# psipred/DMPfold2

Measured on AMD Instinct MI355X. Metric: structures/s at L=300, N_seq=2000, 10 iters+100 min, higher is better.
Workload: dtype f32 with full-width operands on the bf16 matrix cores (option precision = 2): convolution operands split exactly into 3 bf16 pieces (24 significand bits), the 6 piece products above 2^-24 accumulated in f32 by v_mfma_f32_32x32x16_bf16; vertical GRU the same way (3 bf16 pieces per operand, 6 products

## Files before the change

### dmpfold2_amd/csrc/api.hip

```cpp
#include "common.h"
#include <atomic>
#include "conv_bf16.h"
#include "conv_f16.h"
#include <cstdarg>
#include <cstdio>
#include <cstring>
#include <cmath>

namespace dmp {

static thread_local char g_err[512] = "";

void set_error(const char* fmt, ...) {
  va_list ap;
  va_start(ap, fmt);
  vsnprintf(g_err, sizeof(g_err), fmt, ap);
  va_end(ap);
}

int hip_fail(hipError_t e, const char* what, const char* file, int line) {
  set_error("HIP error %d (%s) at %s:%d: %s", (int)e, hipGetErrorString(e), file, line, what);
  return DMP_ERR_HIP;
}

// ... 208 lines not shown
        sc = std::ldexp(1.0f, std::max(-40, std::min(40, 15 - e)));
      }
      W.blk[k - 1].x_scale = sc;
      const std::string p = "resnet." + std::to_string(k);
      bound += 2.0f * reach(H[p + ".layer1.norm.weight"], H[p + ".layer1.norm.bias"]);
    }
  }
  for (int k = 1; k <= NBLOCK; ++k) {
    const std::string p = "resnet." + std::to_string(k);
    BlockW& B = W.blk[k - 1];
    const auto& w = H[p + ".layer1.lin.weight"];
    std::vector<float> pk((size_t)512 * 128 * 25);
    for (int split = 0; split < CONV_SPLIT; ++split)
      for (int chunk = 0; chunk < CW / CONV_CC; ++chunk)
        for (int tap = 0; tap < 25; ++tap)
          for (int cc = 0; cc < CONV_CC; ++cc)
            for (int m = 0; m < 128; ++m) {
              const int och = split * 128 + m, ich = chunk * CONV_CC + cc;
              pk[((((size_t)split * (CW / CONV_CC) + chunk) * 25 + tap) * CONV_CC + cc) * 128 + m] =
                  w[((size_t)och * 128 + ich) * 25 + tap];
            }
    if ((rc = upload(pool, bytes, &B.wpack, pk))) return rc;
    {
      const std::vector<uint16_t> q = pack_conv_weights_bf16(w.data());
      if ((rc = dev_alloc(pool, bytes, &B.wq, (int64_t)q.size()))) return rc;
      DMP_HIP(hipMemcpy(B.wq, q.data(), sizeof(uint16_t) * q.size(), hipMemcpyHostToDevice));
      const float scale = conv_weight_scale_f16(w.data(), w.size());
      const std::vector<uint16_t> h = pack_conv_weights_f16(w.data(), scale);
      if ((rc = dev_alloc(pool, bytes, &B.wh, (int64_t)h.size()))) return rc;
      DMP_HIP(hipMemcpy(B.wh, h.data(), sizeof(uint16_t) * h.size(), hipMemcpyHostToDevice));
      B.wh_inv_scale = 1.0f / scale;
    }
    if ((rc = upload(pool, bytes, &B.bias, H[p + ".layer1.lin.bias"]))) return rc;
    if ((rc = upload(pool, bytes, &B.gamma, H[p + ".layer1.norm.weight"]))) return rc;
    const auto& beta = H[p + ".layer1.norm.bias"];
    if ((rc = upload(pool, bytes, &B.beta, beta))) return rc;
    const auto& w1 = H[p + ".scSE.cSE.fc.0.weight"];
    const auto& w2 = H[p + ".scSE.cSE.fc.2.weight"];
    std::vector<float> hid(8), gate(128);
    for (int r = 0; r < 8; ++r) {
      float a = 0.f;
      for (int q = 0; q < 128; ++q) a += w1[r * 128 + q] * beta[q];
      hid[r] = a > 0.f ? a : 0.f;
    }
    for (int q = 0; q < 128; ++q) {
      float a = 0.f;
      for (int r = 0; r < 8; ++r) a += w2[q * 8 + r] * hid[r];
      gate[q] = 1.0f / (1.0f + std::exp(-a));
    }
    if ((rc = upload(pool, bytes, &B.cse, gate))) return rc;
    {
      std::vector<float> fc(w1);
      fc.insert(fc.end(), w2.begin(), w2.end());
      if ((rc = upload(pool, bytes, &B.cse_fc, fc))) return rc;
    }
    if ((rc = upload(pool, bytes, &B.sse_w, H[p + ".scSE.sSE.conv.weight"]))) return rc;
    B.sse_b = H[p + ".scSE.sSE.conv.bias"][0];
  }
  if ((rc = upload(pool, bytes, &W.head_w, H["resnet.17.weight"]))) return rc;
  W.head_b[0] = H["resnet.17.bias"][0];
  W.head_b[1] = H["resnet.17.bias"][1];
  return DMP_OK;
}

static int check_ready(dmp_ctx* c, int L, int N) {
  if (!c) { set_error("null context"); return DMP_ERR_ARG; }
  if (L > c->max_L || N > c->max_N) {
    set_error("alignment %d x %d exceeds the context capacity %d x %d", N, L, c->max_N, c->max_L);
    return DMP_ERR_CAPACITY;
  }
  return DMP_OK;
}
static int need_weights(dmp_ctx* c) {
  if (!c->W.ready) { set_error("weights not finalized"); return DMP_ERR_WEIGHTS; }
  return DMP_OK;
}

static int trunk_open(dmp_ctx* c, const float* z0, const float* dmap, int L, hipStream_t s) {
  int rc;
  c->trunk_cur = c->xa;
  c->trunk_oth = c->xb;
  c->xsplit_current = false;
  c->ab_current = false;
  if ((rc = stem_update_padded(c, z0, dmap, L, c->trunk_cur, s, true))) return rc;
  c->xsplit_current = c->conv_mode != 1;
  return DMP_OK;
}

static int trunk_block(dmp_ctx* c, int k, int L, hipStream_t s) {
  int rc;
  {
    static const int depth = getenv("DMP_LANE_DEPTH") ? std::max(1, atoi(getenv("DMP_LANE_DEPTH"))) : 2;
    if (c->lane && c->lane->count >= depth)
      DMP_HIP(hipStreamWaitEvent(s, (hipEvent_t)c->lane->ev[(c->lane->count - depth) % dmp_lane::RING], 0));
  }
  if (c->prof_on && c->prof_n + 2 <= (int)c->prof_ev.size()) {
    DMP_HIP(hipEventRecord((hipEvent_t)c->prof_ev[c->prof_n], s));
  }
  if ((rc = conv5x5_maxout_padded(c, k, c->trunk_cur, L, c->u, c->stats, s, false))) return rc;
  if (c->lane) {
    dmp_lane* ln = c->lane;
    void* e = ln->ev[ln->next];
    ln->next = (ln->next + 1) % dmp_lane::RING;
    DMP_HIP(hipEventRecord((hipEvent_t)e, s));
    ln->last = e;
    ln->count++;
  }
  if (c->prof_on && c->prof_n + 2 <= (int)c->prof_ev.size()) {
    DMP_HIP(hipEventRecord((hipEvent_t)c->prof_ev[c->prof_n + 1], s));
    c->prof_n += 2;
  }
  if ((rc = conv5x5_reduce_stats(c, L, c->stats, s, k))) return rc;
  if ((rc = norm_scse_residual_padded(c, k, c->u, c->stats, c->trunk_cur, L, c->trunk_oth, s, k == NBLOCK))) return rc;
  std::swap(c->trunk_cur, c->trunk_oth);
  return DMP_OK;
}

static int trunk_close(dmp_ctx* c, int L, float* d_conf, float* d_M, hipStream_t s) {
  c->xsplit_current = false;
  return head_gram_padded(c, c->trunk_cur, L, d_conf, d_M, s);
}

static int trunk_pass(dmp_ctx* c, const float* z0, const float* dmap, int L, float* d_conf,
                      float* d_M, hipStream_t s) {
  struct Reset { dmp_ctx* c; ~Reset() { c->xsplit_current = false; } } reset{c};
  int rc;
  if ((rc = trunk_open(c, z0, dmap, L, s))) return rc;
  for (int k = 1; k <= NBLOCK; ++k)
    if ((rc = trunk_block(c, k, L, s))) return rc;
  return trunk_close(c, L, d_conf, d_M, s);
}

static int coords_from_mds(dmp_ctx* c, const float* mat1d, const float* mds, int L, float* d_ca,
                           hipStream_t s) {
  int rc;
  if ((rc = build_embed(mat1d, mds, L, c->emb, s))) return rc;
  if ((rc = gru_bidir(c, 1, c->emb, L, c->seq_a, s))) return rc;
  return coord_fc(c, c->seq_a, L, d_ca, s);
}

__global__ void fault_latch_kernel(int* __restrict__ words, float* __restrict__ coords,
                                   float* __restrict__ conf, int L, ConfLayout lay, int* __restrict__ report) {
  const int f = words[0];
  if (!f) return;
  const int64_t i = (int64_t)blockIdx.x * blockDim.x + threadIdx.x;
  const float nan = __builtin_nanf("");
  if (i < 15 * L) coords[i] = nan;
  if (i < lay.score_off || (i >= lay.score_out && i < lay.align_off) || (i >= lay.ss_off && i < lay.align_off) ||
      (i >= lay.align_out && i < lay.total))
    conf[i] = nan;
  if (i == 0) {
    atomicOr(&words[1], f);
    if (report) *report = f;
  }
}

static int search_reserve(dmp_ctx* c) {
  if (c->opt.search <= 0) return DMP_OK;
  const int mm = c->opt.search_mm > 0 ? c->opt.search_mm : c->max_L;
  int64_t need = 0;
  for (int L = 8; L <= c->max_L; ++L)
    need = std::max<int64_t>(need, (int64_t)search_chunk_entries(L, mm, 0) * search_slot(L, mm).total);
  need += SEARCH_HEAD_BYTES;
  if (c->search_ws && c->search_ws_bytes >= need) return DMP_OK;
  int prev = 0;
  DMP_HIP(hipGetDevice(&prev));
  DMP_HIP(hipSetDevice(c->device));
  void* p = nullptr;
  hipError_t e = hipMalloc(&p, (size_t)need);
  if (e == hipSuccess) e = hipMemset(p, 0, (size_t)SEARCH_HEAD_BYTES);
  if (e == hipSuccess && c->search_ws) e = hipFree(c->search_ws);
  (void)hipSetDevice(prev);
  if (e != hipSuccess) {
    if (p) (void)hipFree(p);
    return hip_fail(e, "search scratch", __FILE__, __LINE__);
  }
  c->bytes += need - c->search_ws_bytes;
  c->search_ws = (unsigned char*)p;
  c->search_ws_bytes = need;
  return DMP_OK;
}

static int passes_reserve(dmp_ctx* c) {
  if (c->pass_ws) return DMP_OK;
  const int64_t need = score_passes_bytes(c->max_L);
  int prev = 0;
  DMP_HIP(hipGetDevice(&prev));
  DMP_HIP(hipSetDevice(c->device));
  void* p = nullptr;
  hipError_t e = hipMalloc(&p, (size_t)need);
  if (e == hipSuccess) e = hipMemset(p, 0, (size_t)score_passes_head_bytes());
  (void)hipSetDevice(prev);
  if (e != hipSuccess) {
    if (p) (void)hipFree(p);
    return hip_fail(e, "pass-score scratch", __FILE__, __LINE__);
  }
  c->bytes += need;
  c->pass_ws = (unsigned char*)p;
  c->pass_ws_bytes = need;
  return DMP_OK;
}

static int ss_reserve(dmp_ctx* c) {
  if (c->ss_ws) return DMP_OK;
  const int64_t need = assign_ss_bytes(c->max_L);
  int prev = 0;
  DMP_HIP(hipGetDevice(&prev));
  DMP_HIP(hipSetDevice(c->device));
// ... 905 lines not shown
    c->vg_index = i;
    c->fe_vgru = i == 0 ? ((n > 1 || (lead->vgru_persist && lead->vgru_persist_ok)) ? 1 : cdiv(maxN + 1, FE_VGRU_STEPS)) : 0;
    c->fe_total = 1 + c->fe_inv + c->fe_vgru + 1;
  }
  return DMP_OK;
}

int dmp_predict_group_riders(dmp_ctx* lead, int n, const uint8_t* const* d_msas, const int* Ns, const int* Ls,
                             float* const* d_outs) {
  DMP_ARG(lead && d_msas && Ns && Ls && d_outs && n >= 1, "bad argument");
  DMP_ARG(lead->vg_leader == lead && lead->fe_next == 0 && lead->vg_riders.empty(),
          "add riders right after dmp_predict_group_vgru, once, before the leader issues a unit");
  DMP_ARG((int)lead->vg_members.size() + n <= 8, "a chain serves at most 8 alignments (%d members + %d riders)",
          (int)lead->vg_members.size(), n);
  int cols = 0, maxN = 0;
  for (dmp_ctx* m : lead->vg_members) { cols += round_up(m->last_L, 32); maxN = std::max(maxN, m->last_N); }
  for (int i = 0; i < n; ++i) {
    DMP_ARG(d_msas[i] && d_outs[i] && Ns[i] >= 1 && Ls[i] >= 8, "bad argument for rider %d", i);
    if (Ls[i] > lead->max_L || Ns[i] > lead->max_N) {
      set_error("rider %d: alignment %d x %d exceeds the context capacity %d x %d", i, Ns[i], Ls[i], lead->max_N, lead->max_L);
      return DMP_ERR_CAPACITY;
    }
    cols += round_up(Ls[i], 32);
    maxN = std::max(maxN, Ns[i]);
  }
  if (cols > lead->vg_cap_cols) {
    set_error("the chain's %d alignment columns exceed the leader's capacity %d", cols, lead->vg_cap_cols);
    return DMP_ERR_CAPACITY;
  }
  for (int i = 0; i < n; ++i) lead->vg_riders.push_back({d_msas[i], Ns[i], Ls[i], d_outs[i]});
  lead->fe_vgru = 1;
  lead->fe_total = 1 + lead->fe_inv + lead->fe_vgru + 1;
  return DMP_OK;
}

int dmp_predict_set_vgru_result(dmp_ctx* ctx, const float* d_vout, void* event) {
  DMP_ARG(ctx && d_vout, "null argument");
  DMP_ARG(ctx->fe_total > 0 && ctx->fe_next == 0 && ctx->vg_leader == nullptr,
          "hand the vertical-GRU result over right after dmp_predict_begin_units, before any unit is issued");
  ctx->ext_vout = d_vout;
  ctx->ext_vout_ev = event;
  ctx->fe_vgru = 0;
  ctx->fe_total = 1 + ctx->fe_inv + 1;
  return DMP_OK;
}

int dmp_predict_next_unit(const dmp_ctx* ctx) {
  if (!ctx) return DMP_UNIT_NONE;
  if (ctx->fe_next == ctx->fe_total - 1 && ctx->vg_leader && ctx->vg_leader != ctx && !vg_done(ctx->vg_leader))
    return DMP_UNIT_WAIT;
  if (ctx->fe_next < ctx->fe_total) return DMP_UNIT_LIGHT;
  if (recycle_gate(const_cast<dmp_ctx*>(ctx), false) == 0) return DMP_UNIT_WAIT;
  if (ctx->passes_done > ctx->run_nloops) return DMP_UNIT_NONE;
  return (ctx->unit_next >= 1 && ctx->unit_next <= NBLOCK) ? DMP_UNIT_CONV : DMP_UNIT_LIGHT;
}

int dmp_predict_issue_unit(dmp_ctx* ctx, void* stream) {
  DMP_ARG(ctx != nullptr, "null context");
  dmp_ctx* c = ctx;
  hipStream_t s = STREAM;
  if (c->fe_next < c->fe_total) return issue_front_end_unit(c, s);
  DMP_ARG(c->passes_done <= c->run_nloops, "all passes of this prediction were already issued");
  {
    const int go = recycle_gate(c, true);
    if (go < 0) return go;
    if (c->passes_done > c->run_nloops) return DMP_OK;
  }
  const int L = c->last_L, pass = c->passes_done, u = c->unit_next;
  int rc = DMP_OK;
  if (u == 0) {
    if (pass > 0) rc = pair_distances(c->ca, L, 1, c->dmap, s);
    if (!rc) rc = trunk_open(c, c->z0, c->dmap, L, s);
  } else if (u <= NBLOCK) {
    rc = trunk_block(c, u, L, s);
  } else {
    rc = trunk_close(c, L, c->conf, c->gram, s);
    if (!rc) rc = eigh_top8(c, c->gram, L, c->mds, s);
    if (!rc) rc = coords_from_mds(c, c->mat1d, c->mds, L, c->ca, s);
    if (!rc && pass == 0 && c->run_refine > 0) rc = refine_coords(c, c->ca, L, c->run_refine, s);
    if (!rc) rc = select_best(c, c->conf, c->ca, L, pass, c->max_passes, s);
    if (!rc && c->run.emit) rc = keep_best_dm(c, L, pass, s);
    if (!rc && c->run.tol_mA > 0) rc = recycle_delta(c, c->ca, L, pass, c->max_passes, s);
  }
  if (rc) { c->xsplit_current = false; return rc; }
  if (u == NBLOCK + 1) { c->unit_next = 0; c->passes_done = pass + 1; }
  else c->unit_next = u + 1;
  return record_unit(c, s);
}

int dmp_ctx_pending(dmp_ctx* ctx) {
  DMP_ARG(ctx != nullptr, "null context");
  if (ctx->unit_seq == 0) return 0;
  hipError_t e = hipEventQuery((hipEvent_t)ctx->unit_ev[(ctx->unit_seq - 1) & 1]);
  if (e == hipSuccess) return 0;
  if (e != hipErrorNotReady) return hip_fail(e, "hipEventQuery", __FILE__, __LINE__);
  if (ctx->unit_seq < 2) return 1;
  e = hipEventQuery((hipEvent_t)ctx->unit_ev[ctx->unit_seq & 1]);
  if (e == hipSuccess) return 1;
  if (e != hipErrorNotReady) return hip_fail(e, "hipEventQuery", __FILE__, __LINE__);
  return 2;
}


static int predict_end_refine(dmp_ctx* ctx, void* stream) {
  DMP_ARG(ctx != nullptr, "null context");
  dmp_ctx* c = ctx;
  DMP_ARG(c->fe_next >= c->fe_total && c->passes_done == c->run_nloops + 1,
          "dmp_predict_end before all passes were issued");
  if (c->end_refined) return DMP_OK;
  hipStream_t s = STREAM;
  const int L = c->last_L;
  int rc;
  DMP_HIP(hipMemcpyAsync(c->best_ca_snapshot, c->best_ca, sizeof(float) * 3 * L,
                         hipMemcpyDeviceToDevice, s));
  if (c->run_refine > 0 && (rc = refine_coords(c, c->best_ca, L, c->run_refine, s))) return rc;
  c->end_refined = true;
  return record_unit(c, s);
}

int dmp_predict_end(dmp_ctx* ctx, float* d_coords, float* d_conf, void* stream) {
  DMP_ARG(ctx && d_coords && d_conf, "null argument");
  dmp_ctx* c = ctx;
  int rc = predict_end_refine(ctx, stream);
  if (rc) return rc;
  hipStream_t s = STREAM;
  const int L = c->last_L;
  rc = ca_to_backbone(c->best_ca, c->best_conf, L, d_coords, d_conf, s);
  if (rc) return rc;
  const int pass_R = c->run.passes ? std::min(c->run_depth + 1, c->max_passes) : 0;
  const ConfLayout lay = conf_layout(L, c->run.emit, c->run.score, c->run.align, c->run.smap, pass_R, c->run.ss);
  if (c->run.emit && (rc = emit_distmap(c, c->best_ca, L, c->passes_done, d_conf + lay.map_off, d_conf + lay.info_off, s))) return rc;
  if (c->run.score && (rc = score_native(c, d_coords, L, d_conf + lay.score_off, s))) return rc;
  if (c->run.smap && (rc = score_map(c, L, d_conf + lay.score_off, d_conf + lay.smap_off, s))) return rc;
  if (pass_R && (rc = score_passes(c, L, pass_R, std::min(c->passes_done, c->max_passes), d_conf + lay.pass_off, s))) return rc;
  if (c->run.ss && (rc = assign_ss(c, d_coords, L, c->run.score ? d_conf + lay.score_off : nullptr, d_conf + lay.ss_off, s))) return rc;
  if (c->run.align && (rc = align_structure(c, d_coords, L, d_conf + lay.align_off, s))) return rc;
  if (c->run.search > 0 && (rc = search_structures(c, d_coords, L, d_conf, lay, s))) return rc;
  hipLaunchKernelGGL(fault_latch_kernel, dim3((unsigned)cdiv64(std::max<int64_t>(15 * L, lay.total), 256)), dim3(256), 0, s,
                     c->seq_abort, d_coords, d_conf, L, lay, c->end_fault_out);
  DMP_LAUNCH_CHECK();
  return DMP_OK;
}

static std::shared_ptr<dmp_lane> lane_create() {
  std::shared_ptr<dmp_lane> l(new dmp_lane(), [](dmp_lane* p) {
    for (void* e : p->ev) (void)hipEventDestroy((hipEvent_t)e);
    delete p;
  });
  for (int i = 0; i < dmp_lane::RING; ++i) {
    hipEvent_t e;
    if (hipEventCreateWithFlags(&e, hipEventDisableTiming) != hipSuccess) return nullptr;
    l->ev.push_back((void*)e);
  }
  return l;
}

int dmp_ctx_share_lane(dmp_ctx* ctx, dmp_ctx* other) {
  DMP_ARG(ctx != nullptr, "null context");
  if (!other) { ctx->lane_hold.reset(); ctx->lane = nullptr; return DMP_OK; }
  DMP_ARG(other != ctx && other->device == ctx->device, "a lane is shared by different contexts of one GPU");
  if (!other->lane_hold) {
    other->lane_hold = lane_create();
    if (!other->lane_hold) { set_error("hipEventCreate failed for the lane"); return DMP_ERR_HIP; }
    other->lane = other->lane_hold.get();
  }
  ctx->lane_hold = other->lane_hold;
  ctx->lane = ctx->lane_hold.get();
  return DMP_OK;
}

int64_t dmp_debug_fetch(dmp_ctx* ctx, const char* name, float* d_dst, int64_t capacity, void* stream) {
  DMP_ARG(ctx && name && d_dst, "null argument");
  const int64_t L = ctx->last_L, N = ctx->last_N;
  const int64_t P = std::min(ctx->passes_done, ctx->max_passes);
  const float* src = nullptr;
  int64_t n = 0;
  const std::string k(name);
  if (k == "w") { src = ctx->w; n = N; }
  else if (k == "contacts") { src = ctx->contacts; n = L * L; }
  else if (k == "mat1d") { src = ctx->mat1d; n = WIDTH * L; }
  else if (k == "conf_means") { src = ctx->conf_means; n = P; }
  else if (k == "ca_pass") { src = ctx->ca_pass; n = P * L * 3; }
  else if (k == "pass_delta") { src = ctx->pass_delta; n = ctx->run.tol_mA > 0 ? P : 0; }
  else if (k == "best_dm") { src = ctx->best_dm; n = ctx->run.emit ? L * L : 0; }
  else if (k == "best_pass") { src = ctx->best_pass; n = 1; }
  else if (k == "best_ca") { src = ctx->best_ca_snapshot; n = L * 3; }
  else if (k == "best_ca_refined") { src = ctx->best_ca; n = L * 3; }
  else if (k == "inv_cov") { src = ctx->cov; n = (int64_t)NS * L * NS * L; }
  else if (k == "mds") { src = ctx->mds; n = L * 8; }
  else if (k == "gram") { src = ctx->gram; n = L * L; }
  else if (k == "vgru_h0" || k == "vgru_h1") {
    const int layer = k == "vgru_h1";
    src = ctx->hT[layer][ctx->vg_maxN & 1];
    n = (int64_t)WIDTH * ctx->vg_ntiles * 32;
  }
  else { set_error("unknown debug tensor %s", name); return DMP_ERR_ARG; }
  if (n > capacity) { set_error("capacity %lld too small for %s (%lld)", (long long)capacity, name, (long long)n); return DMP_ERR_ARG; }
  if (n > 0) DMP_HIP(hipMemcpyAsync(d_dst, src, sizeof(float) * n, hipMemcpyDeviceToDevice, STREAM));
  return n;
}

int dmp_profile_enable(dmp_ctx* ctx, int on, int max_launches) {
  DMP_ARG(ctx != nullptr, "null context");
  ctx->prof_on = on != 0;
  ctx->prof_n = 0;
  while ((int)ctx->prof_ev.size() < 2 * max_launches) {
    hipEvent_t e;
    DMP_HIP(hipEventCreate(&e));
    ctx->prof_ev.push_back((void*)e);
  }
  return DMP_OK;
}


int dmp_profile_conv_intervals(dmp_ctx* ctx, dmp_ctx* ref, float* h_start_ms, float* h_end_ms, int capacity,
                               int* h_launches) {
  DMP_ARG(ctx && ref && h_start_ms && h_end_ms && h_launches, "null argument");
  DMP_ARG(ref->prof_n >= 2, "the reference context has no recorded launch");
  const int n = ctx->prof_n / 2 < capacity ? ctx->prof_n / 2 : capacity;
  hipEvent_t e0 = (hipEvent_t)ref->prof_ev[0];
  for (int i = 0; i < n; ++i) {
    DMP_HIP(hipEventElapsedTime(&h_start_ms[i], e0, (hipEvent_t)ctx->prof_ev[2 * i]));
    DMP_HIP(hipEventElapsedTime(&h_end_ms[i], e0, (hipEvent_t)ctx->prof_ev[2 * i + 1]));
  }
  *h_launches = n;
  return DMP_OK;
}


}
```

### dmpfold2_amd/csrc/common.h

```cpp
#pragma once
#include <hip/hip_runtime.h>
#include <stdint.h>
#include <string>
#include <vector>
#include <map>
#include <algorithm>
#include <memory>
#include "../../include/dmpfold_hip.h"

namespace dmp {

constexpr int WIDTH = 512;
constexpr int HID2 = 256;
constexpr float VGRU_STATE_SCALE = 1024.f;
constexpr int VGRU_CHUNK = 128;
constexpr int VGRU_CHUNK_SMALL = 16;
constexpr int CW = 128;
constexpr int NBLOCK = 16;
constexpr int STEM_OUT = 384;
constexpr int STEM_IN = 955;
constexpr int NS = 21;
constexpr int NUM_DCA = NS * NS + 1;
constexpr int GJ_NB = 128;
constexpr int CONV_TILE = 16;
// ... 147 lines not shown
struct dmp_ctx {
  int device = 0;
  dmp_lane* lane = nullptr;
  std::shared_ptr<dmp_lane> lane_hold;
  int run_nloops = 0, run_refine = 0;
  int run_depth = 0;
  int max_L = 0, max_N = 0;
  int64_t bytes = 0;
  dmp::Weights W;
  std::vector<void*> allocs;

  uint8_t* msa = nullptr;
  uint32_t* msa_words = nullptr;
  int* nbr_count = nullptr;
  float* w = nullptr;
  double* wsum = nullptr;
  float* colmean = nullptr;
  float* xc = nullptr;
  float* cov = nullptr;
  float* gj_p = nullptr;
  float *gj_c = nullptr, *gj_rt = nullptr;
  void* gj_ev[2] = {nullptr, nullptr};
  int gj_pairs = 1;
  int gj_lookahead = 1;
  int fe_inv_blocks = 6;
  float* contacts = nullptr;
  float* x3 = nullptr;
  double* apc_sums = nullptr;
  float* hT[2][2] = {{nullptr, nullptr}, {nullptr, nullptr}};
  uint16_t* hH[2][2] = {{nullptr, nullptr}, {nullptr, nullptr}};
  uint8_t* vgru_run = nullptr;
  uint8_t* vgru_sync = nullptr;
  uint8_t* vgru_wq = nullptr;
  int vgru_persist = 1;
  bool vgru_persist_ok = false;
  int vgru_debug_drop_wg = 0;
  int vgru_f32 = 2;
  int vg_ntiles = 0, vg_maxN = 0;
  int vg_tile0[8] = {0};
  int vg_cap_cols = 0;
  dmp_ctx* vg_leader = nullptr;
  std::vector<dmp_ctx*> vg_members;
  struct VgRider { const uint8_t* msa; int N, L; float* out; };
  std::vector<VgRider> vg_riders;
  int vg_index = 0;
  bool vg_done_issued = false;
  int vg_waiters = 0;
  void* vg_done_ev = nullptr;
  const float* ext_vout = nullptr;
  void* ext_vout_ev = nullptr;
  std::map<int64_t, void*> vgru_graphs;
  std::map<int, void*> tri_graphs;
  int cluster_local = 1;
  int tridiag_single = 0;
  int tridiag_cluster = 1;
  unsigned long long* tri_gx = nullptr;
  int refine_single = 0;
  int gj_diag_groups = 4;
  int gj_diag_blocked = 0;
  float* vout = nullptr;
  float* seq_g = nullptr;
  float* seq_a = nullptr;
  float* seq_b = nullptr;
  float* emb = nullptr;
  float* mat1d = nullptr;
  unsigned long long* seq_hx = nullptr;
  int* seq_abort = nullptr;
  unsigned long long* refine_gx = nullptr;
  int refine_xcd = 0;
  int seq_xcd0 = 0;
  float* z0 = nullptr;
  float* planes = nullptr;
  int planes_L = 0;
  bool planes_live = false;
  float* dmap = nullptr;
  float* u = nullptr;
  float* xa = nullptr;
  float* xb = nullptr;
  float* xdense = nullptr;
  uint16_t* xsplit = nullptr;
  int conv_mode = 2;
  int act_scaling = 1;
  bool xsplit_current = false;
  bool ab_current = false;
  double* part = nullptr;
  int part_count = 0;
  int conv_tile_bands = 0;
  double* stats = nullptr;
  float* ab = nullptr;
  float* bwd_ws = nullptr;
  int64_t bwd_ws_floats = 0;
  int bwd_w_block = 0;
  float* head0 = nullptr;
  float* head1 = nullptr;
  bool head_current = false;
  float* conf = nullptr;
  float* gram = nullptr;
  double* eig_a = nullptr;
  double* eig_ws = nullptr;
  float* mds = nullptr;
  float* ca = nullptr;
  float* best_ca = nullptr;
  float* best_conf = nullptr;
  float* best_mean = nullptr;
  float* conf_means = nullptr;
  float* ca_pass = nullptr;
  float* best_ca_snapshot = nullptr;
  int passes_done = 0;
  TailOpts opt;
  TailOpts run;
  int gate_pass = 0;
  float* delta_keep = nullptr;
  float* pass_delta = nullptr;
  double* delta_partial = nullptr;
  unsigned* delta_counter = nullptr;
  int* delta_host = nullptr;
  float* best_pass = nullptr;
  float* best_dm = nullptr;
  double* rms_partial = nullptr;
  unsigned* rms_counter = nullptr;
  float* score_pm = nullptr;
  float* score_qn = nullptr;
  int* score_idx = nullptr;
  double* score_hdr = nullptr;
  double* score_rec = nullptr;
  unsigned long long* score_tot = nullptr;
  unsigned* score_ticket = nullptr;
  unsigned* map_cnt = nullptr;
  double* map_partial = nullptr;
  double* map_sums = nullptr;
  unsigned* map_ticket = nullptr;
  float* align_pm = nullptr;
  float* align_qs = nullptr;
  double* align_hdr = nullptr;
  double* align_rec = nullptr;
  int* align_surv = nullptr;
  double* align_btm = nullptr;
  int* align_bali = nullptr;
  unsigned char* align_dir = nullptr;
  unsigned* align_ticket = nullptr;
  unsigned char* search_ws = nullptr;
  int64_t search_ws_bytes = 0;
  int search_last_L = 0, search_last_mm = 0, search_last_C = 0;
  unsigned char* pass_ws = nullptr;
  int64_t pass_ws_bytes = 0;
  unsigned char* ss_ws = nullptr;
  int64_t ss_ws_bytes = 0;
  int* end_fault_out = nullptr;
  bool end_refined = false;
  int unit_next = 0;
  float *trunk_cur = nullptr, *trunk_oth = nullptr;
  void* unit_ev[2] = {nullptr, nullptr};
  void* side_stream = nullptr;
  void* side_ev[2] = {nullptr, nullptr};
  bool fe_side = false;
  long unit_seq = 0;
  int fe_next = 0, fe_total = 0;
  int fe_inv = 0, fe_vgru = 0;
  const uint8_t* run_msa = nullptr;
  const float* run_template = nullptr;
  int last_L = 0, last_N = 0;
  int max_passes = 0;
  bool prof_on = false;
  int prof_n = 0;
  std::vector<void*> prof_ev;
};
// ... 211 lines not shown
```

### dmpfold2_amd/csrc/trunk.hip

```cpp
#include "common.h"
#include <type_traits>
#define CONV_BF16_KERNELS
#include "conv_bf16.h"
#define CONV_F16_KERNELS
#include "conv_f16.h"

#pragma clang fp contract(off)

namespace dmp {

typedef float f32x16 __attribute__((ext_vector_type(16)));

__device__ __forceinline__ float sigmoid_f(float x) { return 1.0f / (1.0f + expf(-x)); }

template <int MODE>
__device__ __forceinline__ void store_pieces(const float (&o)[8], uint16_t* __restrict__ xs, int64_t slot,
                                             int64_t piece_stride, int* __restrict__ fault, float xscale) {
  constexpr int NP = (MODE == 0) ? 2 : 3;
  uint16_t pc[NP][8];
  bool bad = false;
#pragma unroll
  for (int e = 0; e < 8; ++e) {
    if constexpr (MODE == 0) {
      uint16_t p2[2];
// ... 210 lines not shown
    DMP_LAUNCH_CHECK();
    DMP_HIP(hipMemcpyAsync(c->planes + (int64_t)NS * NS * LL, d_contacts, sizeof(float) * LL, hipMemcpyDeviceToDevice, s));
    planes = c->planes;
  }
  c->planes_L = L;
  c->planes_live = planes != nullptr;
  hipLaunchKernelGGL(stem_static_kernel, dim3((unsigned)cdiv64(LL, 64)), dim3(256), 0, s, W.stemT, W.stem_b,
                     d_mat1d, planes, L, d_z0);
  DMP_LAUNCH_CHECK();
  return DMP_OK;
}

__global__ __launch_bounds__(256) void stem_maxout_kernel(const float* __restrict__ z0,
                                                          const float* __restrict__ wd,
                                                          const float* __restrict__ dmap, int64_t LL,
                                                          float* __restrict__ u, double* __restrict__ part) {
  __shared__ double red[2][4];
  const int64_t p = (int64_t)blockIdx.x * 256 + threadIdx.x;
  const int g = blockIdx.y;
  double s1 = 0.0, s2 = 0.0;
  if (p < LL) {
    const float d = dmap[p];
    const float v0 = z0[(int64_t)(3 * g) * LL + p] + wd[3 * g] * d;
    const float v1 = z0[(int64_t)(3 * g + 1) * LL + p] + wd[3 * g + 1] * d;
    const float v2 = z0[(int64_t)(3 * g + 2) * LL + p] + wd[3 * g + 2] * d;
    const float v = fmaxf(fmaxf(v0, v1), v2);
    u[(int64_t)g * LL + p] = v;
    s1 = (double)v;
    s2 = s1 * s1;
  }
  s1 = wave_sum_f64(s1);
  s2 = wave_sum_f64(s2);
  if ((threadIdx.x & 63) == 0) { red[0][threadIdx.x >> 6] = s1; red[1][threadIdx.x >> 6] = s2; }
  __syncthreads();
  if (threadIdx.x < 2) {
    const double t = ((red[threadIdx.x][0] + red[threadIdx.x][1]) + red[threadIdx.x][2]) + red[threadIdx.x][3];
    part[((int64_t)blockIdx.x * CW + g) * 2 + threadIdx.x] = t;
  }
}

__global__ __launch_bounds__(64) void stats_reduce_kernel(const double* __restrict__ part, int nparts,
                                                          double* __restrict__ stats, double count,
                                                          const float* __restrict__ gamma,
                                                          const float* __restrict__ beta,
                                                          float* __restrict__ ab) {
  const int c = blockIdx.x;
  double s1 = 0.0, s2 = 0.0;
  for (int t = threadIdx.x; t < nparts; t += 64) {
    s1 += part[((int64_t)t * CW + c) * 2 + 0];
    s2 += part[((int64_t)t * CW + c) * 2 + 1];
  }
  for (int off = 32; off > 0; off >>= 1) {
    s1 += __shfl_xor(s1, off, 64);
    s2 += __shfl_xor(s2, off, 64);
  }
  if (threadIdx.x == 0) {
    stats[c * 2 + 0] = s1;
    stats[c * 2 + 1] = s2;
    if (ab) {
      const double mean = s1 / count;
      double var = s2 / count - mean * mean;
      var = var < 0.0 ? 0.0 : var;
      const float invstd = (float)(1.0 / sqrt(var + 1e-5));
      const float alpha = invstd * gamma[c];
      ab[c * 2 + 0] = alpha;
      ab[c * 2 + 1] = beta[c] - (float)mean * alpha;
    }
  }
}

__global__ void norm_coeff_kernel(const double* __restrict__ stats, double count,
                                  const float* __restrict__ gamma, const float* __restrict__ beta,
                                  float* __restrict__ ab) {
  const int c = threadIdx.x;
  const double mean = stats[c * 2] / count;
  double var = stats[c * 2 + 1] / count - mean * mean;
  var = var < 0.0 ? 0.0 : var;
  const float invstd = (float)(1.0 / sqrt(var + 1e-5));
  const float alpha = invstd * gamma[c];
  ab[c * 2 + 0] = alpha;
  ab[c * 2 + 1] = beta[c] - (float)mean * alpha;
}

template <int SPLIT>
__global__ __launch_bounds__(256) void stem_norm_kernel(const float* __restrict__ u,
                                                        const float* __restrict__ ab, int L, int P,
                                                        float* __restrict__ xpad, uint16_t* __restrict__ xs,
                                                        int* __restrict__ fault, float xscale) {
  const int y = blockIdx.y, cgp = blockIdx.z;
  const int x = blockIdx.x * 256 + threadIdx.x;
  if (x >= P) return;
  const int yy = y - 2, xx = x - 2;
  const bool inside = yy >= 0 && yy < L && xx >= 0 && xx < L;
  if (SPLIT < 0 && !inside) return;
  const int64_t PP = (int64_t)P * P, LL = (int64_t)L * L;
  float o[8];
#pragma unroll
  for (int e = 0; e < 8; ++e) {
    const int c = cgp * 8 + e;
    o[e] = 0.f;
    if (inside) {
      o[e] = u[(int64_t)c * LL + (int64_t)yy * L + xx] * ab[c * 2] + ab[c * 2 + 1];
      xpad[(int64_t)c * PP + (int64_t)y * P + x] = o[e];
    }
  }
  if constexpr (SPLIT == 0) store_pieces<0>(o, xs, (int64_t)cgp * PP + (int64_t)y * P + x, 16 * PP, fault, xscale);
  if constexpr (SPLIT == 2) store_pieces<2>(o, xs, (int64_t)cgp * PP + (int64_t)y * P + x, 16 * PP, fault, 1.0f);
}

int stem_update_padded(dmp_ctx* c, const float* d_z0, const float* d_dmap, int L, float* d_xpad,
                       hipStream_t s, bool split) {
  const Weights& W = c->W;
  const int64_t LL = (int64_t)L * L;
  const int P = act_pitch(L);
  const unsigned nblk = (unsigned)cdiv64(LL, 256);
  hipLaunchKernelGGL(stem_maxout_kernel, dim3(nblk, CW), dim3(256), 0, s, d_z0,
                     W.stem_wd, d_dmap, LL, c->u, c->part);
  DMP_LAUNCH_CHECK();
  hipLaunchKernelGGL(stats_reduce_kernel, dim3(CW), dim3(64), 0, s, c->part, (int)nblk, c->stats, (double)LL,
                     W.stem_gamma, W.stem_beta, c->ab);
  DMP_LAUNCH_CHECK();
  const dim3 grid(cdiv(P, 256), P, 16);
  const int mode = (split && c->conv_mode != 1) ? c->conv_mode : -1;
  if (mode == 0)
    hipLaunchKernelGGL(stem_norm_kernel<0>, grid, dim3(256), 0, s, c->u, c->ab, L, P, d_xpad, c->xsplit, c->seq_abort,
                       c->act_scaling ? W.blk[0].x_scale : 1.0f);
  else if (mode == 2)
    hipLaunchKernelGGL(stem_norm_kernel<2>, grid, dim3(256), 0, s, c->u, c->ab, L, P, d_xpad, c->xsplit, c->seq_abort, 1.0f);
  else
    hipLaunchKernelGGL(stem_norm_kernel<-1>, grid, dim3(256), 0, s, c->u, c->ab, L, P, d_xpad, (uint16_t*)nullptr,
                       c->seq_abort, 1.0f);
  DMP_LAUNCH_CHECK();
  return DMP_OK;
}

constexpr int HALO = CONV_TILE + 4;
constexpr int IN_PITCH = 24;
constexpr int NTAP = 25;
constexpr int MCH = 128;
constexpr int NCHUNK = CW / CONV_CC;
constexpr int W_STAGE = NTAP * CONV_CC * MCH;
constexpr int IN_STAGE = CONV_CC * HALO * IN_PITCH;

template <bool IDX>
__global__ __launch_bounds__(256, 2) void conv5x5_maxout_kernel(const float* __restrict__ xpad,
                                                                const float* __restrict__ wpack,
                                                                const float* __restrict__ bias, int L,
                                                                int P, int tiles, int nwork,
                                                                float* __restrict__ u,
                                                                double* __restrict__ part,
                                                                uint8_t* __restrict__ idx) {
  __shared__ __attribute__((aligned(16))) float smem[2 * W_STAGE + 2 * IN_STAGE];
  float (*w_lds)[W_STAGE] = reinterpret_cast<float (*)[W_STAGE]>(smem);
  float (*in_lds)[IN_STAGE] = reinterpret_cast<float (*)[IN_STAGE]>(smem + 2 * W_STAGE);
  constexpr int IP = IN_PITCH;
  const int id = blockIdx.x;
  const int per = gridDim.x >> 3;
  const int work = (id & 7) * per + (id >> 3);
  if (work >= nwork) return;
  const int tile = work >> 2, split = work & 3;
  const int ty0 = (tile / tiles) * CONV_TILE, tx0 = (tile % tiles) * CONV_TILE;

  const int tid = threadIdx.x, lane = tid & 63, wave = tid >> 6;
  const int kk = lane >> 5, li = lane & 31;
  const int64_t PP = (int64_t)P * P;

  const float4* wsrc = reinterpret_cast<const float4*>(wpack + (int64_t)split * NCHUNK * W_STAGE);
  int in_off[4], in_dst[4];
  bool in_ok[4];
#pragma unroll
  for (int e = 0; e < 4; ++e) {
    const int idx = tid + e * 256;
    in_ok[e] = idx < CONV_CC * HALO * HALO;
    const int idc = in_ok[e] ? idx : 0;
    const int cc = idc / (HALO * HALO), rem = idc % (HALO * HALO);
    const int yy = rem / HALO, xx = rem % HALO;
    in_off[e] = (int)(cc * PP + (int64_t)(ty0 + yy) * P + tx0 + xx);
    in_dst[e] = cc * HALO * IP + yy * IP + xx;
  }
  float ireg[4];
  auto prefetch = [&](int chunk) {
    const float4* ws = wsrc + (int64_t)chunk * (W_STAGE / 4);
    const float* xs = xpad + (int64_t)chunk * CONV_CC * PP;
    typedef __attribute__((address_space(1))) const void* gptr_t;
    typedef __attribute__((address_space(3))) void* lptr_t;
    float* dst = w_lds[(chunk & 1)] + (size_t)wave * 256;
#pragma unroll
    for (int e = 0; e < 6; ++e)
      __builtin_amdgcn_global_load_lds((gptr_t)(ws + tid + e * 256), (lptr_t)(dst + e * 1024), 16, 0, 0);
    if (wave == 0)
      __builtin_amdgcn_global_load_lds((gptr_t)(ws + tid + 6 * 256), (lptr_t)(dst + 6 * 1024), 16, 0, 0);
#pragma unroll
    for (int e = 0; e < 4; ++e) ireg[e] = xs[in_off[e]];
  };
  auto commit = [&](int buf) {
#pragma unroll
    for (int e = 0; e < 4; ++e)
      if (in_ok[e]) in_lds[buf][in_dst[e]] = ireg[e];
  };

  int b_off[2];
#pragma unroll
  for (int q = 0; q < 2; ++q) {
    const int nb = 2 * wave + q;
    const int y = (nb >> 1) * 4 + (li >> 3), x = (nb & 1) * 8 + (li & 7);
    b_off[q] = kk * HALO * IP + y * IP + x;
  }
  const int a_off = kk * MCH + li;

  f32x16 acc[4][2];
#pragma unroll
  for (int mb = 0; mb < 4; ++mb)
#pragma unroll
    for (int q = 0; q < 2; ++q)
#pragma unroll
// ... 38 lines not shown
#pragma unroll
      for (int q = 0; q < 2; ++q) {
        float v = acc[mb][q][4 * g4] + bsp[cl];
        int win = 0;
        if constexpr (IDX) {
#pragma unroll
          for (int e = 1; e < 4; ++e) {
            const float t = acc[mb][q][4 * g4 + e] + bsp[cl + e];
            if (t > v) { v = t; win = e; }
          }
        } else {
          v = fmaxf(v, acc[mb][q][4 * g4 + 1] + bsp[cl + 1]);
          v = fmaxf(v, acc[mb][q][4 * g4 + 2] + bsp[cl + 2]);
          v = fmaxf(v, acc[mb][q][4 * g4 + 3] + bsp[cl + 3]);
        }
        const int nb = 2 * wave + q;
        const int y = ty0 + (nb >> 1) * 4 + (li >> 3), x = tx0 + (nb & 1) * 8 + (li & 7);
        if (y < L && x < L) {
          if constexpr (IDX) idx[(int64_t)gch * LL + (int64_t)y * L + x] = (uint8_t)win;
          u[(int64_t)gch * LL + (int64_t)y * L + x] = v;
          s1 += v;
          s2 += v * v;
        }
      }
#pragma unroll
      for (int off = 16; off > 0; off >>= 1) {
        s1 += __shfl_xor(s1, off, 32);
        s2 += __shfl_xor(s2, off, 32);
      }
      if (li == 0) {
        const int chl = (cl >> 2);
        sred[(wave * 32 + chl) * 2 + 0] = s1;
        sred[(wave * 32 + chl) * 2 + 1] = s2;
      }
    }
  __syncthreads();
  if (tid < 64) {
    const int chl = tid >> 1, which = tid & 1;
    double t = 0.0;
#pragma unroll
    for (int wv = 0; wv < 4; ++wv) t += (double)sred[(wv * 32 + chl) * 2 + which];
    part[((int64_t)tile * CW + split * 32 + chl) * 2 + which] = t;
  }
}

int conv5x5_reduce_stats(dmp_ctx* c, int L, double* d_stats, hipStream_t s, int block) {
  const int nparts = c->part_count;
  if (block > 0) {
    const BlockW& B = c->W.blk[block - 1];
    hipLaunchKernelGGL(stats_reduce_kernel, dim3(CW), dim3(64), 0, s, c->part, nparts, d_stats,
                       (double)L * (double)L, B.gamma, B.beta, c->ab);
    c->ab_current = true;
  } else {
    hipLaunchKernelGGL(stats_reduce_kernel, dim3(CW), dim3(64), 0, s, c->part, nparts, d_stats, 1.0,
                       (const float*)nullptr, (const float*)nullptr, (float*)nullptr);
  }
  DMP_LAUNCH_CHECK();
  return DMP_OK;
}

template <int MODE>
__global__ __launch_bounds__(256) void act_split_kernel(const float* __restrict__ xpad, int P,
                                                        uint16_t* __restrict__ xs, int* __restrict__ fault,
                                                        float xscale) {
  const int y = blockIdx.y, cgp = blockIdx.z;
  const int x = blockIdx.x * 256 + threadIdx.x;
  if (x >= P) return;
  const int64_t PP = (int64_t)P * P;
  float o[8];
#pragma unroll
  for (int e = 0; e < 8; ++e) o[e] = xpad[(int64_t)(cgp * 8 + e) * PP + (int64_t)y * P + x];
  store_pieces<MODE>(o, xs, (int64_t)cgp * PP + (int64_t)y * P + x, 16 * PP, fault, xscale);
}

int act_split(dmp_ctx* c, const float* d_xpad, int L, int block, hipStream_t s) {
  const int P = act_pitch(L);
  dim3 grid(cdiv(P, 256), P, 16);
  if (c->conv_mode == 2)
    hipLaunchKernelGGL(act_split_kernel<2>, grid, dim3(256), 0, s, d_xpad, P, c->xsplit, c->seq_abort, 1.0f);
  else
    hipLaunchKernelGGL(act_split_kernel<0>, grid, dim3(256), 0, s, d_xpad, P, c->xsplit, c->seq_abort,
                       c->act_scaling ? c->W.blk[block - 1].x_scale : 1.0f);
  DMP_LAUNCH_CHECK();
  return DMP_OK;
}

int trunk_kernel_attrs(dmp_ctx* c) {
  static bool done[64] = {};
  if (c->device >= 0 && c->device < 64 && done[c->device]) return DMP_OK;
  auto lds = [](const void* k, int bytes) { return hipFuncSetAttribute(k, hipFuncAttributeMaxDynamicSharedMemorySize, bytes); };
  DMP_HIP(lds((const void*)conv5x5_bf16x6_kernel<8>, convq_lds_bytes<8>()));
  DMP_HIP(lds((const void*)conv5x5_bf16x6_kernel<4>, convq_lds_bytes<4>()));
  DMP_HIP(lds((const void*)conv5x5_f16x3_kernel<8>, convh_lds_bytes<8>()));
  DMP_HIP(lds((const void*)conv5x5_f16x3_kernel<4>, convh_lds_bytes<4>()));
  if (c->device >= 0 && c->device < 64) done[c->device] = true;
  return DMP_OK;
}

int conv5x5_maxout_padded(dmp_ctx* c, int block, const float* d_xpad, int L, float* d_u,
                          double* d_stats, hipStream_t s, bool reduce) {
  const BlockW& B = c->W.blk[block - 1];
  const int tiles = act_tiles(L), P = act_pitch(L);
  const int nwork = tiles * tiles * CONV_SPLIT;
  const int grid = round_up(nwork, 8);
  if (c->conv_mode != 1) {
    if (!c->xsplit_current) {
      int rc = act_split(c, d_xpad, L, block, s);
      if (rc) return rc;
    }
    const int bands = c->conv_tile_bands > 0 ? c->conv_tile_bands : conv_split_rows(tiles);
    const float scale = c->act_scaling ? B.wh_inv_scale / B.x_scale : B.wh_inv_scale;
    if (c->conv_mode == 2) {
      if (bands == 2)
        hipLaunchKernelGGL(conv5x5_bf16x6_kernel<4>, dim3(conv_split_grid(tiles, 2)), dim3(256), convq_lds_bytes<4>(), s,
                           c->xsplit, B.wq, B.bias, L, P, tiles, nwork, d_u, c->part);
      else
        hipLaunchKernelGGL(conv5x5_bf16x6_kernel<8>, dim3(conv_split_grid(tiles, 1)), dim3(256), convq_lds_bytes<8>(), s,
                           c->xsplit, B.wq, B.bias, L, P, tiles, nwork, d_u, c->part);
    } else {
      if (bands == 2)
        hipLaunchKernelGGL(conv5x5_f16x3_kernel<4>, dim3(conv_split_grid(tiles, 2)), dim3(256), convh_lds_bytes<4>(), s,
                           c->xsplit, B.wh, B.bias, scale, L, P, tiles, nwork, d_u, c->part);
      else
        hipLaunchKernelGGL(conv5x5_f16x3_kernel<8>, dim3(conv_split_grid(tiles, 1)), dim3(256), convh_lds_bytes<8>(), s,
                           c->xsplit, B.wh, B.bias, scale, L, P, tiles, nwork, d_u, c->part);
    }
    DMP_LAUNCH_CHECK();
    c->part_count = 2 * tiles * tiles;
    return reduce ? conv5x5_reduce_stats(c, L, d_stats, s) : DMP_OK;
  }
  hipLaunchKernelGGL(conv5x5_maxout_kernel<false>, dim3(grid), dim3(256), 0, s, d_xpad, B.wpack, B.bias, L,
                     P, tiles, nwork, d_u, c->part, (uint8_t*)nullptr);
  DMP_LAUNCH_CHECK();
  c->part_count = tiles * tiles;
  return reduce ? conv5x5_reduce_stats(c, L, d_stats, s) : DMP_OK;
}

int conv5x5_maxout_winners(dmp_ctx* c, int block, const float* d_xpad, int L, float* d_u, uint8_t* d_idx, hipStream_t s) {
  const BlockW& B = c->W.blk[block - 1];
  const int tiles = act_tiles(L), P = act_pitch(L);
  const int nwork = tiles * tiles * CONV_SPLIT;
  hipLaunchKernelGGL(conv5x5_maxout_kernel<true>, dim3(round_up(nwork, 8)), dim3(256), 0, s, d_xpad, B.wpack, B.bias, L,
                     P, tiles, nwork, d_u, c->part, d_idx);
  DMP_LAUNCH_CHECK();
  c->part_count = tiles * tiles;
  return DMP_OK;
}

#ifndef NORM_PRIO
#define NORM_PRIO 0
#endif
template <int SPLIT, int HEAD>
__global__ __launch_bounds__(256) void norm_scse_residual_kernel(
    const float* __restrict__ u, const float* __restrict__ ab, const float* __restrict__ cse,
    const float* __restrict__ sse_w, float sse_b, const float* __restrict__ xin, int L, int P,
    float* __restrict__ xout, uint16_t* __restrict__ xs, int* __restrict__ fault, float xscale,
    const float* __restrict__ hw, float hb0, float hb1, float* __restrict__ head0, float* __restrict__ head1) {
  __shared__ float sh_a[CW], sh_b[CW], sh_g[CW], sh_w[CW], sh_h[HEAD ? 2 * CW : 1];
#if NORM_PRIO
  __builtin_amdgcn_s_setprio(NORM_PRIO);
#endif
  if (threadIdx.x < CW) {
    sh_a[threadIdx.x] = ab[threadIdx.x * 2];
    sh_b[threadIdx.x] = ab[threadIdx.x * 2 + 1];
    sh_g[threadIdx.x] = cse[threadIdx.x];
    sh_w[threadIdx.x] = sse_w[threadIdx.x];
  }
  if constexpr (HEAD) sh_h[threadIdx.x] = hw[threadIdx.x];
  __syncthreads();
  const int lane = threadIdx.x & 63, wave = threadIdx.x >> 6;
  const int q = lane >> 4;
  const int y = blockIdx.y;
  const int x = blockIdx.x * 64 + wave * 16 + (lane & 15);
  const bool live = x < L;
  const int xc = live ? x : L - 1;
  const int64_t LL = (int64_t)L * L, PP = (int64_t)P * P;
  const int64_t p = (int64_t)y * L + xc, pp = (int64_t)(y + 2) * P + xc + 2;
  constexpr int QC = CW / 4;
  float yv[QC];
  float dot = 0.f;
#pragma unroll
  for (int i = 0; i < QC; ++i) {
    const int c = q * QC + i;
    yv[i] = u[c * LL + p] * sh_a[c] + sh_b[c];
    dot = fmaf(sh_w[c], yv[i], dot);
  }
  dot += __shfl_xor(dot, 16, 64);
  dot += __shfl_xor(dot, 32, 64);
  const float sg = sigmoid_f(dot + sse_b);
  float h0 = 0.f, h1 = 0.f;
#pragma unroll
  for (int g8 = 0; g8 < QC / 8; ++g8) {
    const int cgp = q * (QC / 8) + g8;
    float o[8];
#pragma unroll
    for (int e = 0; e < 8; ++e) {
      const int c = cgp * 8 + e;
      const float t = yv[g8 * 8 + e] * sh_g[c] + yv[g8 * 8 + e] * sg;
      o[e] = t + xin[c * PP + pp];
      if (live) xout[c * PP + pp] = o[e];
      if constexpr (HEAD) {
        h0 = fmaf(sh_h[c], o[e], h0);
        h1 = fmaf(sh_h[CW + c], o[e], h1);
      }
    }
    if (live) {
      if constexpr (SPLIT == 0) store_pieces<0>(o, xs, (int64_t)cgp * PP + pp, 16 * PP, fault, xscale);
      if constexpr (SPLIT == 2) store_pieces<2>(o, xs, (int64_t)cgp * PP + pp, 16 * PP, fault, 1.0f);
    }
  }
  if constexpr (HEAD) {
    h0 += __shfl_xor(h0, 16, 64);
    h0 += __shfl_xor(h0, 32, 64);
    h1 += __shfl_xor(h1, 16, 64);
    h1 += __shfl_xor(h1, 32, 64);
    if (live && q == 0) {
      head0[(int64_t)y * L + x] = h0 + hb0;
      head1[(int64_t)y * L + x] = h1 + hb1;
    }
  }
}

int norm_scse_residual_padded(dmp_ctx* c, int block, const float* d_u, const double* d_stats,
                              const float* d_xpad_in, int L, float* d_xpad_out, hipStream_t s, bool head) {
  const BlockW& B = c->W.blk[block - 1];
  const Weights& W = c->W;
  const int P = act_pitch(L);
  if (!c->ab_current) {
    hipLaunchKernelGGL(norm_coeff_kernel, dim3(1), dim3(CW), 0, s, d_stats, (double)L * (double)L,
                       B.gamma, B.beta, c->ab);
    DMP_LAUNCH_CHECK();
  }
  c->ab_current = false;
  const int split = (c->conv_mode != 1 && c->xsplit_current && block < NBLOCK) ? c->conv_mode : -1;
  const float xscale = (c->act_scaling && block < NBLOCK) ? c->W.blk[block].x_scale : 1.0f;
  dim3 grid(cdiv(L, 64), L);
#define NORM_LAUNCH(S, H)                                                                              \
  hipLaunchKernelGGL((norm_scse_residual_kernel<S, H>), grid, dim3(256), 0, s, d_u, c->ab, B.cse, B.sse_w, \
                     B.sse_b, d_xpad_in, L, P, d_xpad_out, c->xsplit, c->seq_abort, xscale, W.head_w,   \
                     W.head_b[0], W.head_b[1], c->head0, c->head1)
  if (head) NORM_LAUNCH(-1, 1);
  else if (split == 0) NORM_LAUNCH(0, 0);
  else if (split == 2) NORM_LAUNCH(2, 0);
  else NORM_LAUNCH(-1, 0);
#undef NORM_LAUNCH
  DMP_LAUNCH_CHECK();
  c->head_current = head;
  return DMP_OK;
}

__global__ __launch_bounds__(256) void head_planes_kernel(const float* __restrict__ xpad,
                                                          const float* __restrict__ hw, float b0, float b1,
                                                          int L, int P, float* __restrict__ head0,
                                                          float* __restrict__ head1) {
  __shared__ float sw[2 * CW];
  sw[threadIdx.x] = hw[threadIdx.x];
  __syncthreads();
  const int i = blockIdx.y;
  const int j = blockIdx.x * 256 + threadIdx.x;
  if (j >= L) return;
  const int64_t PP = (int64_t)P * P;
  const float* px = xpad + (int64_t)(i + 2) * P + j + 2;
  float p0[4], p1[4];
#pragma unroll
  for (int q = 0; q < 4; ++q) {
    p0[q] = 0.f; p1[q] = 0.f;
#pragma unroll 8
    for (int k = 0; k < CW / 4; ++k) {
      const int c = q * (CW / 4) + k;
      const float v = px[c * PP];
      p0[q] = fmaf(sw[c], v, p0[q]);
      p1[q] = fmaf(sw[CW + c], v, p1[q]);
    }
  }
  head0[(int64_t)i * L + j] = ((p0[0] + p0[1]) + (p0[2] + p0[3])) + b0;
  head1[(int64_t)i * L + j] = ((p1[0] + p1[1]) + (p1[2] + p1[3])) + b1;
}

__global__ __launch_bounds__(256) void head_conf_kernel(const float* __restrict__ head1, int L,
                                                        float* __restrict__ conf) {
  __shared__ double red[256];
  const int i = blockIdx.x;
  double rsum = 0.0;
  for (int j = threadIdx.x; j < L; j += 256) rsum += (double)head1[(int64_t)i * L + j];
  const double total = block_tree_sum_f64<256>(rsum, red);
  if (threadIdx.x == 0) conf[i] = (float)(total / (double)L);
}

__global__ __launch_bounds__(256) void gram_kernel(const float* __restrict__ h0, int L,
                                                   float* __restrict__ M) {
  const int i = blockIdx.y;
  const int j = blockIdx.x * 256 + threadIdx.x;
  if (j >= L) return;
  auto dm = [&](int a, int b) {
    return distmap_entry(h0[(int64_t)a * L + b], h0[(int64_t)b * L + a]);
  };
  const float d0j = dm(0, j), di0 = dm(i, 0), dij = dm(i, j);
  const float t = d0j * d0j + di0 * di0;
  M[(int64_t)i * L + j] = 0.5f * (t - dij * dij);
}

int head_gram_padded(dmp_ctx* c, const float* d_xpad, int L, float* d_conf, float* d_M,
                     hipStream_t s) {
  const Weights& W = c->W;
  const int P = act_pitch(L);
  if (!c->head_current) {
    hipLaunchKernelGGL(head_planes_kernel, dim3(cdiv(L, 256), L), dim3(256), 0, s, d_xpad, W.head_w, W.head_b[0],
                       W.head_b[1], L, P, c->head0, c->head1);
    DMP_LAUNCH_CHECK();
  }
  c->head_current = false;
  hipLaunchKernelGGL(head_conf_kernel, dim3(L), dim3(256), 0, s, c->head1, L, d_conf);
  DMP_LAUNCH_CHECK();
  hipLaunchKernelGGL(gram_kernel, dim3(cdiv(L, 256), L), dim3(256), 0, s, c->head0, L, d_M);
  DMP_LAUNCH_CHECK();
  return DMP_OK;
}

}

#ifdef CQ_CLOCK_STAMPS
extern "C" int dmp_debug_conv_clock(unsigned long long* host, int blocks) {
  if (!host || blocks < 1 || blocks > dmp::CQ_STAMP_BLOCKS) return -1;
  if (hipDeviceSynchronize() != hipSuccess) return -1;
  return hipMemcpyFromSymbol(host, HIP_SYMBOL(dmp::cq_clock_stamps), sizeof(unsigned long long) * 2 * blocks) == hipSuccess ? 0 : -1;
}
#endif
```

Baseline: 4.231.

## Keep trunk activations only as bf16 pieces, dropping the f32 padded plane

In precision mode 2 the stem no longer writes the f32 padded activation plane. A new norm/SCSE/residual kernel rebuilds the residual input from the three bf16 pieces and writes updated pieces back in place, with the head projection reduced in shared memory on the last block. This removes the f32 plane write and read each block, trading them for piece reconstruction arithmetic. It relies on the three-piece sum being exact and on no other consumer needing the f32 plane. Debug accessors for head planes and xsplit are also added.

```diff
diff --git a/dmpfold2_amd/csrc/api.hip b/dmpfold2_amd/csrc/api.hip
--- a/dmpfold2_amd/csrc/api.hip
+++ b/dmpfold2_amd/csrc/api.hip
@@ -314,7 +314,8 @@
   c->trunk_oth = c->xb;
   c->xsplit_current = false;
   c->ab_current = false;
-  if ((rc = stem_update_padded(c, z0, dmap, L, c->trunk_cur, s, true))) return rc;
+  c->pieces_only = c->conv_mode == 2;
+  if ((rc = stem_update_padded(c, z0, dmap, L, c->trunk_cur, s, true))) { c->pieces_only = false; return rc; }
   c->xsplit_current = c->conv_mode != 1;
   return DMP_OK;
 }
@@ -350,12 +351,13 @@
 
 static int trunk_close(dmp_ctx* c, int L, float* d_conf, float* d_M, hipStream_t s) {
   c->xsplit_current = false;
+  c->pieces_only = false;
   return head_gram_padded(c, c->trunk_cur, L, d_conf, d_M, s);
 }
 
 static int trunk_pass(dmp_ctx* c, const float* z0, const float* dmap, int L, float* d_conf,
                       float* d_M, hipStream_t s) {
-  struct Reset { dmp_ctx* c; ~Reset() { c->xsplit_current = false; } } reset{c};
+  struct Reset { dmp_ctx* c; ~Reset() { c->xsplit_current = false; c->pieces_only = false; } } reset{c};
   int rc;
   if ((rc = trunk_open(c, z0, dmap, L, s))) return rc;
   for (int k = 1; k <= NBLOCK; ++k)
@@ -1427,7 +1429,7 @@
     if (!rc && c->run.emit) rc = keep_best_dm(c, L, pass, s);
     if (!rc && c->run.tol_mA > 0) rc = recycle_delta(c, c->ca, L, pass, c->max_passes, s);
   }
-  if (rc) { c->xsplit_current = false; return rc; }
+  if (rc) { c->xsplit_current = false; c->pieces_only = false; return rc; }
   if (u == NBLOCK + 1) { c->unit_next = 0; c->passes_done = pass + 1; }
   else c->unit_next = u + 1;
   return record_unit(c, s);
@@ -1534,6 +1536,15 @@
   else if (k == "inv_cov") { src = ctx->cov; n = (int64_t)NS * L * NS * L; }
   else if (k == "mds") { src = ctx->mds; n = L * 8; }
   else if (k == "gram") { src = ctx->gram; n = L * L; }
+  else if (k == "head0" || k == "head1") {
+    src = k == "head0" ? ctx->head0 : ctx->head1;
+    n = (int64_t)ctx->trunk_L * ctx->trunk_L;
+  }
+  else if (k == "xsplit") {
+    const int64_t P = act_pitch(ctx->trunk_L);
+    src = reinterpret_cast<const float*>(ctx->xsplit);
+    n = ctx->conv_mode == 1 ? 0 : (ctx->conv_mode == 2 ? 3 : 2) * (int64_t)CW * P * P / 2;
+  }
   else if (k == "vgru_h0" || k == "vgru_h1") {
     const int layer = k == "vgru_h1";
     src = ctx->hT[layer][ctx->vg_maxN & 1];
diff --git a/dmpfold2_amd/csrc/common.h b/dmpfold2_amd/csrc/common.h
--- a/dmpfold2_amd/csrc/common.h
+++ b/dmpfold2_amd/csrc/common.h
@@ -253,6 +253,8 @@
   int conv_mode = 2;
   int act_scaling = 1;
   bool xsplit_current = false;
+  bool pieces_only = false;
+  int trunk_L = 0;
   bool ab_current = false;
   double* part = nullptr;
   int part_count = 0;
diff --git a/dmpfold2_amd/csrc/trunk.hip b/dmpfold2_amd/csrc/trunk.hip
--- a/dmpfold2_amd/csrc/trunk.hip
+++ b/dmpfold2_amd/csrc/trunk.hip
@@ -316,7 +316,7 @@
   ab[c * 2 + 1] = beta[c] - (float)mean * alpha;
 }
 
-template <int SPLIT>
+template <int SPLIT, bool PLANE = true>
 __global__ __launch_bounds__(256) void stem_norm_kernel(const float* __restrict__ u,
                                                         const float* __restrict__ ab, int L, int P,
                                                         float* __restrict__ xpad, uint16_t* __restrict__ xs,
@@ -335,7 +335,7 @@
     o[e] = 0.f;
     if (inside) {
       o[e] = u[(int64_t)c * LL + (int64_t)yy * L + xx] * ab[c * 2] + ab[c * 2 + 1];
-      xpad[(int64_t)c * PP + (int64_t)y * P + x] = o[e];
+      if constexpr (PLANE) xpad[(int64_t)c * PP + (int64_t)y * P + x] = o[e];
     }
   }
   if constexpr (SPLIT == 0) store_pieces<0>(o, xs, (int64_t)cgp * PP + (int64_t)y * P + x, 16 * PP, fault, xscale);
@@ -359,12 +359,16 @@
   if (mode == 0)
     hipLaunchKernelGGL(stem_norm_kernel<0>, grid, dim3(256), 0, s, c->u, c->ab, L, P, d_xpad, c->xsplit, c->seq_abort,
                        c->act_scaling ? W.blk[0].x_scale : 1.0f);
+  else if (mode == 2 && c->pieces_only)
+    hipLaunchKernelGGL((stem_norm_kernel<2, false>), grid, dim3(256), 0, s, c->u, c->ab, L, P, (float*)nullptr, c->xsplit,
+                       c->seq_abort, 1.0f);
   else if (mode == 2)
     hipLaunchKernelGGL(stem_norm_kernel<2>, grid, dim3(256), 0, s, c->u, c->ab, L, P, d_xpad, c->xsplit, c->seq_abort, 1.0f);
   else
     hipLaunchKernelGGL(stem_norm_kernel<-1>, grid, dim3(256), 0, s, c->u, c->ab, L, P, d_xpad, (uint16_t*)nullptr,
                        c->seq_abort, 1.0f);
   DMP_LAUNCH_CHECK();
+  c->trunk_L = L;
   return DMP_OK;
 }
 
@@ -569,6 +573,7 @@
     hipLaunchKernelGGL(act_split_kernel<0>, grid, dim3(256), 0, s, d_xpad, P, c->xsplit, c->seq_abort,
                        c->act_scaling ? c->W.blk[block - 1].x_scale : 1.0f);
   DMP_LAUNCH_CHECK();
+  c->trunk_L = L;
   return DMP_OK;
 }
 
@@ -708,6 +713,87 @@
   }
 }
 
+__device__ __forceinline__ float join3_bf16(uint32_t h0, uint32_t h1, uint32_t h2) {
+  const float a = __builtin_bit_cast(float, h0), b = __builtin_bit_cast(float, h1), c = __builtin_bit_cast(float, h2);
+  const float s = (a + b) + c;
+  return s == 0.f ? a : s;
+}
+__device__ __forceinline__ void join_pieces(const uint4 (&r)[3], float (&x)[8]) {
+  const uint32_t w[3][4] = {{r[0].x, r[0].y, r[0].z, r[0].w}, {r[1].x, r[1].y, r[1].z, r[1].w}, {r[2].x, r[2].y, r[2].z, r[2].w}};
+#pragma unroll
+  for (int e = 0; e < 8; e += 2) {
+    x[e] = join3_bf16(w[0][e >> 1] << 16, w[1][e >> 1] << 16, w[2][e >> 1] << 16);
+    x[e + 1] = join3_bf16(w[0][e >> 1] & 0xFFFF0000u, w[1][e >> 1] & 0xFFFF0000u, w[2][e >> 1] & 0xFFFF0000u);
+  }
+}
+
+template <int HEAD>
+__global__ __launch_bounds__(256) void norm_scse_residual_pieces_kernel(
+    const float* __restrict__ u, const float* __restrict__ ab, const float* __restrict__ cse,
+    const float* __restrict__ sse_w, float sse_b, int L, int P, uint16_t* xs, int* __restrict__ fault,
+    const float* __restrict__ hw, float hb0, float hb1, float* __restrict__ head0, float* __restrict__ head1) {
+  __shared__ float sh_dot[4][64];
+  __shared__ float sh_head[HEAD ? 2 : 1][4][64];
+  const int lane = threadIdx.x & 63;
+  const int q = __builtin_amdgcn_readfirstlane(threadIdx.x >> 6);
+  const int64_t LL = (int64_t)L * L, PP = (int64_t)P * P;
+  const int64_t p = (int64_t)blockIdx.x * 64 + lane;
+  const bool live = p < LL;
+  const int64_t pc = live ? p : LL - 1;
+  const int y = (int)(pc / L), x = (int)(pc - (int64_t)y * L);
+  const int64_t pp = live ? (int64_t)(y + 2) * P + x + 2 : 0;
+  constexpr int QC = CW / 4, NG = QC / 8;
+  uint4* xs4 = reinterpret_cast<uint4*>(xs);
+  uint4 r[NG][3];
+#pragma unroll
+  for (int g8 = 0; g8 < NG; ++g8)
+#pragma unroll
+    for (int k = 0; k < 3; ++k) r[g8][k] = xs4[k * 16 * PP + (int64_t)(q * NG + g8) * PP + pp];
+  float yv[QC];
+#pragma unroll
+  for (int i = 0; i < QC; ++i) yv[i] = u[(q * QC + i) * LL + pc];
+  __builtin_amdgcn_sched_barrier(0);
+  float dot = 0.f;
+#pragma unroll
+  for (int i = 0; i < QC; ++i) {
+    const int c = q * QC + i;
+    yv[i] = yv[i] * ab[c * 2] + ab[c * 2 + 1];
+    dot = fmaf(sse_w[c], yv[i], dot);
+  }
+  sh_dot[q][lane] = dot;
+  __syncthreads();
+  const float sg = sigmoid_f(((sh_dot[0][lane] + sh_dot[1][lane]) + (sh_dot[2][lane] + sh_dot[3][lane])) + sse_b);
+  float h0 = 0.f, h1 = 0.f;
+#pragma unroll
+  for (int g8 = 0; g8 < NG; ++g8) {
+    const int cgp = q * NG + g8;
+    float xr[8], o[8];
+    join_pieces(r[g8], xr);
+#pragma unroll
+    for (int e = 0; e < 8; ++e) {
+      const int c = cgp * 8 + e;
+      const float t = yv[g8 * 8 + e] * cse[c] + yv[g8 * 8 + e] * sg;
+      o[e] = t + xr[e];
+      if constexpr (HEAD) {
+        h0 = fmaf(hw[c], o[e], h0);
+        h1 = fmaf(hw[CW + c], o[e], h1);
+      }
+    }
+    if constexpr (!HEAD) {
+      if (live) store_pieces<2>(o, xs, (int64_t)cgp * PP + pp, 16 * PP, fault, 1.0f);
+    }
+  }
+  if constexpr (HEAD) {
+    sh_head[0][q][lane] = h0;
+    sh_head[1][q][lane] = h1;
+    __syncthreads();
+    if (live && q == 0) {
+      head0[p] = ((sh_head[0][0][lane] + sh_head[0][1][lane]) + (sh_head[0][2][lane] + sh_head[0][3][lane])) + hb0;
+      head1[p] = ((sh_head[1][0][lane] + sh_head[1][1][lane]) + (sh_head[1][2][lane] + sh_head[1][3][lane])) + hb1;
+    }
+  }
+}
+
 int norm_scse_residual_padded(dmp_ctx* c, int block, const float* d_u, const double* d_stats,
                               const float* d_xpad_in, int L, float* d_xpad_out, hipStream_t s, bool head) {
   const BlockW& B = c->W.blk[block - 1];
@@ -719,6 +805,19 @@
     DMP_LAUNCH_CHECK();
   }
   c->ab_current = false;
+  c->trunk_L = L;
+  if (c->pieces_only && c->conv_mode == 2 && c->xsplit_current) {
+    const dim3 pgrid((unsigned)cdiv64((int64_t)L * L, 64));
+#define NORM_PIECES_LAUNCH(H)                                                                                    \
+  hipLaunchKernelGGL((norm_scse_residual_pieces_kernel<H>), pgrid, dim3(256), 0, s, d_u, c->ab, B.cse, B.sse_w, \
+                     B.sse_b, L, P, c->xsplit, c->seq_abort, W.head_w, W.head_b[0], W.head_b[1], c->head0, c->head1)
+    if (head) NORM_PIECES_LAUNCH(1);
+    else NORM_PIECES_LAUNCH(0);
+#undef NORM_PIECES_LAUNCH
+    DMP_LAUNCH_CHECK();
+    c->head_current = head;
+    return DMP_OK;
+  }
   const int split = (c->conv_mode != 1 && c->xsplit_current && block < NBLOCK) ? c->conv_mode : -1;
   const float xscale = (c->act_scaling && block < NBLOCK) ? c->W.blk[block].x_scale : 1.0f;
   dim3 grid(cdiv(L, 64), L);
@@ -797,6 +896,7 @@
     DMP_LAUNCH_CHECK();
   }
   c->head_current = false;
+  c->trunk_L = L;
   hipLaunchKernelGGL(head_conf_kernel, dim3(L), dim3(256), 0, s, c->head1, L, d_conf);
   DMP_LAUNCH_CHECK();
   hipLaunchKernelGGL(gram_kernel, dim3(cdiv(L, 256), L), dim3(256), 0, s, c->head0, L, d_M);
```

Result: no change. 4.205 (-0.6%).
